# ai2cm/pace

Hardware: AMD Instinct MI355X
Metric: cell-updates/s per acoustic substep (d_sw+riem3), C192x79L; % HBM roofline (higher is better)
Workload: dtype f64; 1 GPU; C192x79L one tile per GPU, d_sw + riem_solver3 acoustic substep, fp64; cells_per_tile=2912256, tiles=1, parallelism=tile-per-gpu x1, halo_exchange=none, launch=eager, streams=one stream

## Files before the change

pace_amd/csrc/k_fxadv.hip:

```cpp
#include "common.h"
#include "kernels.h"

typedef SplitBox FxBox;

__device__ __forceinline__ double contra(double v1, double v2, double cosa, double rsin2) {
  return (v1 - v2 * cosa) * rsin2;
}

__device__ __forceinline__ void fx_vt_edges_point(const Geo& g, const Met& m, const real* vc, const real* ut, real* vt, int i, int j,
                                                  int k) {
  if (i > g.ni - 2 || j > g.nj - 2) return;
  const long c = IDX3(g, i, j, k);
  const long c2 = IDX2(g, i, j);
  if (j == g.js || j == g.je + 1) {
    const double v = vc[c];
    vt[c] = (v > 0.0) ? (v / m.sin_sg4[c2 - g.sj]) : (v / m.sin_sg2[c2]);
    return;
  }
  const bool strip = (i == g.is - 1 || i == g.is || i == g.ie || i == g.ie + 1);
  if (strip && j >= g.js + 2 && j <= g.je - 1) {
    const double ub = 0.25 * (ut[c - g.sj] + ut[c + 1 - g.sj] + ut[c] + ut[c + 1]);
    vt[c] = contra(vc[c], ub, m.cosa_v[c2], 1.0);
  }
}

__device__ __forceinline__ void fx_ut_edges_corners_point(const Geo& g, const Met& m, const real* uc, const real* vc, real* ut,
                                                          const real* vt, int i, int j, int k) {
  if (i < 1 || j < 1 || i > g.ni - 2 || j > g.nj - 2) return;
  const long c = IDX3(g, i, j, k);
  const long c2 = IDX2(g, i, j);
  const int sj = g.sj;
  const bool rows = (j == g.js - 1 || j == g.js || j == g.je || j == g.je + 1);
  if (rows && i >= g.is + 2 && i <= g.ie - 1) {
    const double vb = 0.25 * (vt[c - 1] + vt[c] + vt[c - 1 + sj] + vt[c + sj]);
    ut[c] = contra(uc[c], vb, m.cosa_u[c2], 1.0);
    return;
  }
  if (rows && (i == g.is + 1 || i == g.ie)) {
    const double cu = m.cosa_u[c2];
    double damp, val;
    if (i == g.is + 1 && (j == g.js - 1 || j == g.je)) {
      const double cv = m.cosa_v[c2 - 1];
      damp = 1.0 / (1.0 - 0.0625 * cu * cv);
      val = (uc[c] - 0.25 * cu * (vt[c - 1 + sj] + vt[c + sj] + vt[c] + vc[c - 1] -
                                  0.25 * cv * (ut[c - 1] + ut[c - 1 - sj] + ut[c - sj]))) * damp;
    } else if (i == g.is + 1) {
      const double cv = m.cosa_v[c2 - 1 + sj];
      damp = 1.0 / (1.0 - 0.0625 * cu * cv);
      val = (uc[c] - 0.25 * cu * (vt[c - 1] + vt[c] + vt[c + sj] + vc[c - 1 + sj] -
                                  0.25 * cv * (ut[c - 1] + ut[c - 1 + sj] + ut[c + sj]))) * damp;
    } else if (j == g.js - 1 || j == g.je) {
      const double cv = m.cosa_v[c2];
      damp = 1.0 / (1.0 - 0.0625 * cu * cv);
      val = (uc[c] - 0.25 * cu * (vt[c + sj] + vt[c - 1 + sj] + vt[c - 1] + vc[c] -
                                  0.25 * cv * (ut[c + 1] + ut[c + 1 - sj] + ut[c - sj]))) * damp;
    } else {
      const double cv = m.cosa_v[c2 + sj];
      damp = 1.0 / (1.0 - 0.0625 * cu * cv);
      val = (uc[c] - 0.25 * cu * (vt[c] + vt[c - 1] + vt[c - 1 + sj] + vc[c + sj] -
                                  0.25 * cv * (ut[c + 1] + ut[c + 1 + sj] + ut[c + sj]))) * damp;
    }
    ut[c] = val;
    return;
  }
}

__device__ __forceinline__ void fx_vt_corners_point(const Geo& g, const Met& m, const real* uc, const real* vc, const real* ut,
                                                    real* vt, int i, int j, int k) {
  if (i < 1 || j < 1 || i > g.ni - 2 || j > g.nj - 2) return;
  const bool cols = (i == g.is - 1 || i == g.is || i == g.ie || i == g.ie + 1);
  if (!cols || !(j == g.js + 1 || j == g.je)) return;
  const long c = IDX3(g, i, j, k);
  const long c2 = IDX2(g, i, j);
  const int sj = g.sj;
  const double cv = m.cosa_v[c2];
  double damp, val;
  if (j == g.js + 1 && (i == g.is - 1 || i == g.ie)) {
    const double cu = m.cosa_u[c2 - sj];
    damp = 1.0 / (1.0 - 0.0625 * cu * cv);
    val = (vc[c] - 0.25 * cv * (ut[c + 1 - sj] + ut[c + 1] + ut[c] + uc[c - sj] -
                                0.25 * cu * (vt[c - sj] + vt[c - 1 - sj] + vt[c - 1]))) * damp;
  } else if (j == g.js + 1) {
    const double cu = m.cosa_u[c2 + 1 - sj];
    damp = 1.0 / (1.0 - 0.0625 * cu * cv);
    val = (vc[c] - 0.25 * cv * (ut[c - sj] + ut[c] + ut[c + 1] + uc[c + 1 - sj] -
                                0.25 * cu * (vt[c - sj] + vt[c + 1 - sj] + vt[c + 1]))) * damp;
  } else if (i == g.ie + 1 || i == g.is) {
    const double cu = m.cosa_u[c2 + 1];
    damp = 1.0 / (1.0 - 0.0625 * cu * cv);
    val = (vc[c] - 0.25 * cv * (ut[c] + ut[c - sj] + ut[c + 1 - sj] + uc[c + 1] -
                                0.25 * cu * (vt[c + sj] + vt[c + 1 + sj] + vt[c + 1]))) * damp;
  } else {
    const double cu = m.cosa_u[c2];
    damp = 1.0 / (1.0 - 0.0625 * cu * cv);
    val = (vc[c] - 0.25 * cv * (ut[c + 1] + ut[c + 1 - sj] + ut[c - sj] + uc[c] -
                                0.25 * cu * (vt[c + sj] + vt[c - 1 + sj] + vt[c - 1]))) * damp;
  }
  vt[c] = val;
}

struct FxStrips {
  Regions b, c, d;
};
__device__ __forceinline__ bool strip_point(const Regions& R, int p, int& i, int& j) {
  for (int q = 0; q < R.n; ++q) {
    const int w = R.ie[q] - R.ib[q] + 1, h = R.je[q] - R.jb[q] + 1;
    if (p < w * h) {
      j = R.jb[q] + p / w;
      i = R.ib[q] + p % w;
      return true;
    }
    p -= w * h;
  }
  return false;
}
__device__ __forceinline__ int strip_count(const Regions& R) {
  int n = 0;
  for (int q = 0; q < R.n; ++q) n += (R.ie[q] - R.ib[q] + 1) * (R.je[q] - R.jb[q] + 1);
  return n;
}
struct FxFramePointA {
  long c;
  bool xedge, umain, vmain;
  double u0, u_s, u1_s, u1, v0, v_1, v_1s, vs, s3, s1, cu, ru, cv, rv;
  __device__ __forceinline__ void load(const Geo& g, const Met& m, const real* __restrict__ uc, const real* __restrict__ vc, bool on, int i,
                                       int j, int k) {
    const long c2 = IDX2(g, i, j);
    c = IDX3(g, i, j, k);
    const int sj = g.sj;
    xedge = on && (i == g.is || i == g.ie + 1);
    umain = on && !xedge && i >= g.is - 1 && i <= g.ie + 2 && !(j == g.js - 1 || j == g.js || j == g.je || j == g.je + 1);
    vmain = on && j >= g.js - 1 && j <= g.je + 2;
    u0 = u_s = u1_s = u1 = v0 = v_1 = v_1s = vs = s3 = s1 = cu = ru = cv = rv = 0.0;
    if (xedge || umain || vmain) u0 = uc[c];
    if (umain || vmain) v0 = vc[c];
    if (xedge) s3 = m.sin_sg3[c2 - 1], s1 = m.sin_sg1[c2];
    if (umain) v_1 = vc[c - 1], v_1s = vc[c - 1 + sj], vs = vc[c + sj], cu = m.cosa_u[c2], ru = m.rsin_u[c2];
    if (vmain) u_s = uc[c - sj], u1_s = uc[c + 1 - sj], u1 = uc[c + 1], cv = m.cosa_v[c2], rv = m.rsin_v[c2];
  }
  __device__ __forceinline__ void finish(real* ut, real* vt) const {
    if (xedge) {
      ut[c] = (u0 > 0.0) ? (u0 / s3) : (u0 / s1);
    } else if (umain) {
      const double vb = 0.25 * (v_1 + v0 + v_1s + vs);
      ut[c] = contra(u0, vb, cu, ru);
    }
    if (vmain) {
      const double ub = 0.25 * (u_s + u1_s + u0 + u1);
      vt[c] = contra(v0, ub, cv, rv);
    }
  }
};
struct FxFramePointF {
  long c;
  bool do_x, do_y;
  double u, v, rdxa_m, rdxa_0, dy, sg3_m, sg1_0, rdya_m, rdya_0, dx, sg4_m, sg2_0, cxa, cya;
  __device__ __forceinline__ void load(const Geo& g, const Met& m, const real* ut, const real* vt, const real* cx_acc, const real* cy_acc,
                                       bool on, int i, int j, int k) {
    const long c2 = IDX2(g, i, j);
    c = c2 + (long)k * g.sk;
    const int sj = g.sj;
    do_x = on && i >= g.is && i <= g.ie + 1, do_y = on && j >= g.js && j <= g.je + 1;
    u = v = rdxa_m = rdxa_0 = dy = sg3_m = sg1_0 = rdya_m = rdya_0 = dx = sg4_m = sg2_0 = cxa = cya = 0.0;
    if (do_x) {
      u = ut[c], rdxa_m = m.rdxa[c2 - 1], rdxa_0 = m.rdxa[c2], dy = m.dy[c2], sg3_m = m.sin_sg3[c2 - 1], sg1_0 = m.sin_sg1[c2];
      if (cx_acc) cxa = cx_acc[c];
    }
    if (do_y) {
      v = vt[c], rdya_m = m.rdya[c2 - sj], rdya_0 = m.rdya[c2], dx = m.dx[c2], sg4_m = m.sin_sg4[c2 - sj], sg2_0 = m.sin_sg2[c2];
      if (cy_acc) cya = cy_acc[c];
    }
  }
  __device__ __forceinline__ void finish(double dt, real* crx, real* cry, real* xfx, real* yfx, real* cx_acc, real* cy_acc) const {
    if (do_x) {
      double cr;
      if (u > 0.0) {
        cr = dt * u * rdxa_m;
        xfx[c] = dy * dt * u * sg3_m;
      } else {
        cr = dt * u * rdxa_0;
        xfx[c] = dy * dt * u * sg1_0;
      }
      crx[c] = cr;
      if (cx_acc) cx_acc[c] = cxa + cr;
    }
    if (do_y) {
      double cr;
      if (v > 0.0) {
        cr = dt * v * rdya_m;
        yfx[c] = dx * dt * v * sg4_m;
      } else {
        cr = dt * v * rdya_0;
        yfx[c] = dx * dt * v * sg2_0;
      }
      cry[c] = cr;
      if (cy_acc) cy_acc[c] = cya + cr;
    }
  }
};
#ifndef FX_NB
#define FX_NB 1
#endif

#ifndef FX_NT
#define FX_NT 1024
#endif
#ifndef FX_MIN_WGS
#define FX_MIN_WGS (512 * 1024 / FX_NT)
#endif
#ifndef FX_ATTR
#define FX_ATTR
#endif
template <int FXC>
__global__ void __launch_bounds__(FX_NT) FX_ATTR k_fxadv_fused(Geo g, Met m, const real* __restrict__ uc, const real* __restrict__ vc, real* ut, real* vt,
                                                      real* __restrict__ crx, real* __restrict__ cry, real* __restrict__ xfx,
                                                      real* __restrict__ yfx, double dt, real* __restrict__ cx_acc,
                                                      real* __restrict__ cy_acc, FxBox box, int contra_out, Regions A, FxStrips S,
                                                      int nframe, int nbx, FxWindHalo wh) {
  const int tid = (int)threadIdx.x;
  int b = (int)blockIdx.x;
  if (b < nframe) {
    const int k = b;
    int i, j;
    const int na = strip_count(A);
    if (wh.u_out != nullptr)
      for (int p = tid, n = wind_halo_points(g); p < n; p += FX_NT) wind_halo_copy_point(g, p, k, wh.u, wh.v, wh.u_out, wh.v_out);
    for (int p0 = tid; p0 < na; p0 += FX_NT * FX_NB) {
      FxFramePointA P[FX_NB];
#pragma unroll
      for (int q = 0; q < FX_NB; ++q) {
        int pi = 0, pj = 0;
        const bool on = strip_point(A, p0 + q * FX_NT, pi, pj) && pi <= g.ni - 2 && pj <= g.nj - 2;
        P[q].load(g, m, uc, vc, on, on ? pi : 1, on ? pj : 1, k);
      }
#pragma unroll
      for (int q = 0; q < FX_NB; ++q) P[q].finish(ut, vt);
    }
    __threadfence_block();
    __syncthreads();
    for (int p = tid, n = strip_count(S.b); p < n; p += FX_NT)
      if (strip_point(S.b, p, i, j)) fx_vt_edges_point(g, m, vc, ut, vt, i, j, k);
    __threadfence_block();
    __syncthreads();
    for (int p = tid, n = strip_count(S.c); p < n; p += FX_NT)
      if (strip_point(S.c, p, i, j)) fx_ut_edges_corners_point(g, m, uc, vc, ut, vt, i, j, k);
    __threadfence_block();
    __syncthreads();
    for (int p = tid, n = strip_count(S.d); p < n; p += FX_NT)
      if (strip_point(S.d, p, i, j)) fx_vt_corners_point(g, m, uc, vc, ut, vt, i, j, k);
    __threadfence_block();
    __syncthreads();
    for (int p0 = tid; p0 < na; p0 += FX_NT * FX_NB) {
      FxFramePointF P[FX_NB];
#pragma unroll
      for (int q = 0; q < FX_NB; ++q) {
        int pi = 0, pj = 0;
        const bool on = strip_point(A, p0 + q * FX_NT, pi, pj);
        P[q].load(g, m, ut, vt, cx_acc, cy_acc, on, on ? pi : 1, on ? pj : 1, k);
      }
#pragma unroll
      for (int q = 0; q < FX_NB; ++q) P[q].finish(dt, crx, cry, xfx, yfx, cx_acc, cy_acc);
    }
    return;
  }
  b -= nframe;
#ifdef PACE_EMU
  const int chunk = b / nbx, bxp = b - chunk * nbx;
#else
  const int seg = nbx / 8;
  const int chunk = b / nbx, r = b - chunk * nbx;
  const int bxp = (r & 7) * seg + (r >> 3);
#endif
  const long p = (long)bxp * FX_NT + tid;
  const int j = (int)(p / g.sj);
  const int i = (int)(p - (long)j * g.sj);
  if (i < box.i0 || i > box.i1 || j < box.j0 || j > box.j1) return;
  const int k0 = chunk * FXC;
  const long c2 = IDX2(g, i, j);
  const int sj = g.sj;
  const double rdxa_m = m.rdxa[c2 - 1], rdxa_0 = m.rdxa[c2], dy = m.dy[c2], sg3_m = m.sin_sg3[c2 - 1], sg1_0 = m.sin_sg1[c2];
  const double rdya_m = m.rdya[c2 - sj], rdya_0 = m.rdya[c2], dx = m.dx[c2], sg4_m = m.sin_sg4[c2 - sj], sg2_0 = m.sin_sg2[c2];
  const double cosa_u = m.cosa_u[c2], rsin_u = m.rsin_u[c2], cosa_v = m.cosa_v[c2], rsin_v = m.rsin_v[c2];
#pragma unroll
  for (int t = 0; t < FXC; ++t) {
    const int k = k0 + t;
    if (k >= g.nk) break;
    const long c = c2 + (long)k * g.sk;
    const double uc0 = uc[c], vc0 = vc[c];
    const double vb = 0.25 * (vc[c - 1] + vc0 + vc[c - 1 + sj] + vc[c + sj]);
    const double ub = 0.25 * (uc[c - sj] + uc[c + 1 - sj] + uc0 + uc[c + 1]);
    const double u = contra(uc0, vb, cosa_u, rsin_u);
    const double v = contra(vc0, ub, cosa_v, rsin_v);
    if (contra_out) ut[c] = u, vt[c] = v;
    double cr;
    if (u > 0.0) {
      cr = dt * u * rdxa_m;
      xfx[c] = dy * dt * u * sg3_m;
    } else {
      cr = dt * u * rdxa_0;
      xfx[c] = dy * dt * u * sg1_0;
    }
    crx[c] = cr;
    if (cx_acc) cx_acc[c] = cx_acc[c] + cr;
    if (v > 0.0) {
      cr = dt * v * rdya_m;
      yfx[c] = dx * dt * v * sg4_m;
    } else {
      cr = dt * v * rdya_0;
      yfx[c] = dx * dt * v * sg2_0;
    }
    cry[c] = cr;
    if (cy_acc) cy_acc[c] = cy_acc[c] + cr;
  }
}

static void fxadv_frame_regions(const Geo& g, bool has_box, Regions& A, FxStrips& S) {
  if (has_box) {
    add_region(A, 0, g.ni - 2, 0, g.js + 1);
    add_region(A, 0, g.ni - 2, g.je - 1, g.nj - 2);
    add_region(A, 0, g.is + 1, g.js + 2, g.je - 2);
    add_region(A, g.ie - 1, g.ni - 2, g.js + 2, g.je - 2);
  } else {
    add_region(A, 0, g.ni - 2, 0, g.nj - 2);
  }
  add_region(S.b, 0, g.ni - 2, g.js, g.js);
  add_region(S.b, 0, g.ni - 2, g.je + 1, g.je + 1);
  add_region(S.b, g.is - 1, g.is, g.js + 2, g.je - 1);
  add_region(S.b, g.ie, g.ie + 1, g.js + 2, g.je - 1);
  add_region(S.c, g.is + 1, g.ie, g.js - 1, g.js);
  add_region(S.c, g.is + 1, g.ie, g.je, g.je + 1);
  add_region(S.d, g.is - 1, g.ie + 1, g.js + 1, g.js + 1);
  add_region(S.d, g.is - 1, g.ie + 1, g.je, g.je);
}

int launch_fxadv(const Geo& g, const Met& m, const real* uc, const real* vc, real* crx, real* cry,
                 real* xfx, real* yfx, real* ut, real* vt, double dt, real* cx_acc, real* cy_acc,
                 hipStream_t st, int part, int contra_out, FxWindHalo* wind_halo) {
  FxBox box{g.is + 2, g.ie - 2, g.js + 2, g.je - 2, part};
  const bool has_box = box.i1 >= box.i0 && box.j1 >= box.j0;
  if (!has_box) box.i1 = box.i0 - 1, box.j1 = box.j0 - 1;
  if (part == 1 && !has_box) return PACE_OK;
  Regions A{};
  FxStrips S{};
  if (part != 1) fxadv_frame_regions(g, has_box, A, S);
  const int nframe = (part != 1) ? g.nk : 0;
  unsigned nbx = (unsigned)(((long)g.sj * g.nj + FX_NT - 1) / FX_NT);
#ifndef PACE_EMU
  nbx = (nbx + 7) / 8 * 8;
#endif
  const bool interior = has_box && part != 2;
  int ch = 8;
  while (ch > 1 && nbx * (unsigned)((g.nk + ch - 1) / ch) < (unsigned)FX_MIN_WGS) ch >>= 1;
  const unsigned nint = interior ? nbx * (unsigned)((g.nk + ch - 1) / ch) : 0u;
  if (nframe + nint == 0) return PACE_OK;
  FxWindHalo wcopy{nullptr, nullptr, nullptr, nullptr, false};
  if (wind_halo != nullptr && nframe > 0) wcopy = *wind_halo, wind_halo->done = true;
#define FX_GO(CH)                                                                                                                            \
  hipLaunchKernelGGL(k_fxadv_fused<CH>, dim3((unsigned)nframe + nint), dim3(FX_NT), 0, st, g, m, uc, vc, ut, vt, crx, cry, xfx, yfx, dt, cx_acc, \
                     cy_acc, box, contra_out, A, S, nframe, (int)nbx, wcopy)
  if (ch == 8) FX_GO(8);
  else if (ch == 4) FX_GO(4);
  else if (ch == 2) FX_GO(2);
  else FX_GO(1);
#undef FX_GO
  PACE_CHECK_LAUNCH();
  return PACE_OK;
}
```

pace_amd/csrc/kernels.h:

```cpp
#pragma once
#include "common.h"

struct FxWindHalo {
  const real *u, *v;
  real *u_out, *v_out;
  bool done;
};
int launch_fxadv(const Geo& g, const Met& m, const real* uc, const real* vc, real* crx, real* cry,
                 real* xfx, real* yfx, real* ut, real* vt, double dt, real* cx_acc, real* cy_acc,
                 hipStream_t st, int part = 0, int contra_out = 0, FxWindHalo* wind_halo = nullptr);
__device__ __forceinline__ void wind_halo_copy_point(const Geo& g, int p, int k, const real* __restrict__ u, const real* __restrict__ v,
                                                     real* __restrict__ u_out, real* __restrict__ v_out) {
  const int nsouth = g.js, nnorth = g.nj - 1 - g.je, nmid = g.je - g.js + 1, nwest = g.is, neast = g.ni - 1 - g.ie;
  const int rows = (nsouth + nnorth) * g.ni;
  int i, j;
  if (p < rows) {
    const int r = p / g.ni;
    i = p - r * g.ni, j = r < nsouth ? r : g.je + 1 + (r - nsouth);
  } else {
    p -= rows;
    const int w = nwest + neast, r = p / w, c = p - r * w;
    if (r >= nmid) return;
    j = g.js + r, i = c < nwest ? c : g.ie + 1 + (c - nwest);
  }
  const long ch = IDX3(g, i, j, k);
  const bool in_i = i >= g.is && i <= g.ie, in_j = j >= g.js && j <= g.je;
  if (!(in_i && (in_j || j == g.je + 1))) u_out[ch] = u[ch];
  if (!((in_i || i == g.ie + 1) && in_j)) v_out[ch] = v[ch];
}
__host__ __device__ __forceinline__ int wind_halo_points(const Geo& g) {
  return (g.js + g.nj - 1 - g.je) * g.ni + (g.je - g.js + 1) * (g.is + g.ni - 1 - g.ie);
}
int launch_fvtp2d(const Geo& g, const Met& m, const real* q, const real* crx, const real* cry,
                  const real* xfx, const real* yfx, real* fx, real* fy, const real* xmf,
                  const real* ymf, int hord, int nlev, hipStream_t st);
struct FvDamp {
  const real* damp_k;
  const real* nord_k;
  const real* mass;
  real* fx2o;
  real* fy2o;
  int nmax, mass_given;
  real* qout;
  const real* amass;
  real* dw;
  real* heat_s;
  real* diss_est;
  const real* damp_w_k;
  const real* ke_bg_k;
  double dt;
  real* accx;
  real* accy;
  const real* add2d;
  real* u_upd;
  real* v_upd;
  const real* ke;
  real* u_out;
  real* v_out;
};

int launch_transport(const Geo& g, const Met& m, const real* q, const real* crx, const real* cry, const real* xfx,
                     const real* yfx, real* fx, real* fy, const real* xmf, const real* ymf, int hord, int nlev,
                     int dmode, int epi, const FvDamp& dp, hipStream_t st);
int launch_transport_scalars3(const Geo& g, const Met& m, const real* w, const real* q_con, const real* pt, const real* crx,
                              const real* cry, const real* xfx, const real* yfx, const real* xmf, const real* ymf, int nlev,
                              const FvDamp& dpw, const FvDamp& dpq, const FvDamp& dpt, hipStream_t st);
int launch_transport_lean(const Geo& g, const Met& m, const real* q, const real* crx, const real* cry, const real* xfx,
                          const real* yfx, real* fx, real* fy, const real* xu, const real* yu, int hord, int nlev, int dmode,
                          int epi, const FvDamp& dp, hipStream_t st);

struct DswWinds {
  const real *rel_vort, *u, *v, *ke, *vort_b;
  real *u_out, *v_out, *heat_source;
  int do_skeb, copy_halo;
  int ke_plus_vort;
  double d_con;
};
bool dsw_scalars_take_winds();
int launch_dsw_scalars_lean(const Geo& g, const Met& m, const real* delp, const real* pt, const real* w, const real* q_con,
                            real* const* outs, const real* crx, const real* cry, const real* xfx, const real* yfx, real* mfx,
                            real* mfy, real* dw, real* heat_s, real* diss_est, const real* kc, int hord, int nmax_v, int nmax_w,
                            int nmax_t, double dt, hipStream_t st, const DswWinds* winds = nullptr);
bool transport_lean_covers(const Geo& g, int hord);

struct FvMet {
  const real *area, *rarea, *dxa, *dya, *dx, *dy, *del6_u, *del6_v;
};
static inline FvMet fv_met(const Met& m) { return FvMet{m.area, m.rarea, m.dxa, m.dya, m.dx, m.dy, m.del6_u, m.del6_v}; }

struct FvTile {
  int bx, by, bz;
};
__device__ __forceinline__ FvTile fv_tile_of_workgroup() {
#ifdef PACE_EMU
  return FvTile{(int)blockIdx.x, (int)blockIdx.y, (int)blockIdx.z};
#else
  const int gx = gridDim.x, gy = gridDim.y, nlev = gridDim.z;
  const int tpl = gx * gy;
  const int b = blockIdx.x + gx * (blockIdx.y + gy * blockIdx.z);
  const int full = (nlev / 8) * 8;
  int lev, t;
  if (b < full * tpl) {
    const int xcd = b & 7, slot = b >> 3;
    lev = (slot / tpl) * 8 + xcd;
    t = slot - (slot / tpl) * tpl;
  } else {
    lev = b / tpl;
    t = b - lev * tpl;
  }
  if (gx >= 3 && gy >= 3) {
    if (t < 4) return FvTile{(t & 1) ? gx - 1 : 0, (t & 2) ? gy - 1 : 0, lev};
    t -= 4;
    const int nsn = 2 * (gx - 2), nwe = 2 * (gy - 2);
    if (t < nsn) return FvTile{1 + (t >> 1), (t & 1) ? gy - 1 : 0, lev};
    t -= nsn;
    if (t < nwe) return FvTile{(t & 1) ? gx - 1 : 0, 1 + (t >> 1), lev};
    t -= nwe;
    return FvTile{1 + t % (gx - 2), 1 + t / (gx - 2), lev};
  }
  return FvTile{t % gx, t / gx, lev};
#endif
}
int launch_delnflux(const Geo& g, const Met& m, int mode, const real* q, real* fx, real* fy,
                    const real* mass, const real* damp_k, const real* nord_k, int nmax, int mass_given,
                    int nlev, hipStream_t st);
int launch_a2b_ord4(const Geo& g, const Met& m, real* qin, real* qout, int k0, int k1, int replace, hipStream_t st);
int launch_a2b_ord4_tiled(const Geo& g, const Met& m, const real* qin, real* qout, int k0, int k1, hipStream_t st);
int launch_a2b_ord4_batch(const Geo& g, const Met& m, const real* const* qin, real* const* qout, const int* k0, const int* k1,
                          int nfields, hipStream_t st);
int64_t dsw_workspace_bytes(const Geo& g);
bool dsw_pingpong_supported(const Geo& g, const pace_dsw_config_t* cfg);
bool dsw_winds_in_scalars(const Geo& g, const pace_dsw_config_t* cfg);
int dsw_prepare(const Geo& g, const pace_column_t* col, void* ws, hipStream_t st);
int launch_d_sw(const Geo& g, const Met& m, const pace_column_t* col, const pace_dsw_config_t* cfg, void* ws,
                real* delpc, real* delp, real* pt, real* u, real* v, real* w, real* uc, real* vc,
                const real* ua, const real* va, real* divgd, real* mfx, real* mfy, real* cx, real* cy,
                real* crx, real* cry, real* xfx, real* yfx, real* q_con, const real* zh,
                real* heat_source, real* diss_est, double dt, int phases, hipStream_t st);
int64_t riem3_workspace_bytes(const Geo& g);
int launch_riem_solver3(const Geo& g, void* ws, int last_call, double dt, const real* cappa, double ptop,
                        const real* zs, const real* wsd, real* delz, const real* q_con, const real* delp,
                        const real* pt, real* zh, real* pe, real* ppe, real* pk3, real* pk, real* peln,
                        real* w, double p_fac, hipStream_t st);
int launch_ppm1d(const Geo& g, const Met& m, int axis, int iord, const real* q, const real* c, real* out, int i0, int j0,
                 int k0, int ni, int nj, int nk, hipStream_t st);
int launch_divergence_damping(const Geo& g, const Met& m, const real* u, const real* v, const real* va, real* vort_b,
                              const real* ua, real* divg_d, real* vc, real* uc, real* delpc, real* ke,
                              const real* rel_vort_agrid, double dt, const real* d2_bg_dev, int kstart, int nonzero_nord,
                              double dddmp, double d4_bg, real* da, real* db, hipStream_t st, bool skip_dead = false,
                              bool ke_by_consumer = false, const int* ddh_tab = nullptr);
bool riem_column_supported(const Geo& g);
int launch_riem_solver3_column(const Geo& g, int last_call, double dt, const real* cappa, double ptop, const real* zs,
                               const real* wsd, real* delz, const real* q_con, const real* delp, const real* pt,
                               real* zh, real* pe, real* ppe, real* pk3, real* pk, real* peln, real* w,
                               double p_fac, hipStream_t st);
int launch_riem_solver_c_column(const Geo& g, double dt2, const real* cappa, double ptop, const real* hs, const real* ws3,
                                const real* ptc, const real* q_con, const real* delpc, real* gz, real* pef,
                                const real* w3, double p_fac, hipStream_t st);
int64_t sim1_workspace_bytes(const Geo& g);
int launch_sim1_solver(const Geo& g, void* ws, int n_halo, double dt, double p_fac, const real* gamma, const real* cp3,
                       real* pe, const real* delta_mass, const real* pm, const real* pem, real* w, real* dz,
                       const real* pt, const real* ws2d, hipStream_t st);
int64_t csw_workspace_bytes(const Geo& g);
int launch_d2a2c_vect(const Geo& g, const Met& m, void* ws, real* uc, real* vc, const real* u, const real* v,
                      real* ua, real* va, real* utc, real* vtc, hipStream_t st);
int launch_c_sw(const Geo& g, const Met& m, void* ws, real* delpc, real* ptc, real* delp, real* pt,
                const real* u, const real* v, real* w, real* uc, real* vc, real* ua, real* va,
                real* ut, real* vt, real* divgd, real* omga, double dt2, int nord, hipStream_t st, int part = 0);
int64_t riemc_workspace_bytes(const Geo& g);
int launch_riem_solver_c(const Geo& g, void* ws, double dt2, const real* cappa, double ptop, const real* hs,
                         const real* ws3, const real* ptc, const real* q_con, const real* delpc, real* gz,
                         real* pef, const real* w3, double p_fac, hipStream_t st);
int64_t updatedzc_workspace_bytes(const Geo& g);
int launch_updatedzc(const Geo& g, const Met& m, void* ws_, const real* dp_ref, const real* zs, const real* ut,
                     const real* vt, real* gz, real* ws, double dt, hipStream_t st);
int64_t updatedzd_workspace_bytes(const Geo& g);
int launch_updatedzd(const Geo& g, const Met& m, void* ws_, const pace_updatedzd_k_t* kc, const real* zs, real* zh,
                     const real* crx, const real* cry, const real* xfx, const real* yfx, real* wsd, double dt,
                     int hord_tm, hipStream_t st);
int launch_gz_from_surface(const Geo& g, const real* zs, const real* delz, real* gz, hipStream_t st);
int launch_scale_copy(const Geo& g, const real* src, real* dst, double factor, int scale, int halo, int nlev,
                      hipStream_t st);
int launch_p_grad_c(const Geo& g, const Met& m, real* uc, real* vc, const real* delpc, const real* pkc,
                    const real* gz, double dt2, hipStream_t st);
int64_t nh_p_grad_workspace_bytes(const Geo& g);
int launch_nh_p_grad(const Geo& g, const Met& m, void* ws_, real* u, real* v, real* pp, real* gz, real* pk3,
                     real* delp, double dt, double ptop, double akap, hipStream_t st);
int launch_edge_pe(const Geo& g, real* pe, const real* delp, double ptop, hipStream_t st);
int launch_pk3_halo(const Geo& g, real* pk3, const real* delp, double ptop, double akap, hipStream_t st);
int launch_ray_fast(const Geo& g, real* u, real* v, real* w, const double* dp, const double* pfull, double dt,
                    double ptop, double rf_cutoff, double tau, int hydrostatic, hipStream_t st);
int64_t del2cubed_workspace_bytes(const Geo& g);
int launch_del2cubed(const Geo& g, const Met& m, void* ws_, real* qdel, double cd, int nmax, hipStream_t st);
int launch_diffusive_heating(const Geo& g, const real* delp, const real* delz, const real* cappa,
                             const real* heat_source, real* pt, double delt_time_factor, int nlev, hipStream_t st);
int launch_halo_copy(const Geo& g, const pace_halo_desc_t* descs, int ndesc, int unpack, hipStream_t st);
int launch_tracer_flux_compute(const Geo& g, const Met& m, const real* cx, const real* cy, real* xfx, real* yfx,
                               hipStream_t st);
int launch_tracer_divide(const Geo& g, real* cxd, real* xfx, real* mfxd, real* cyd, real* yfx, real* mfyd,
                         int n_split, hipStream_t st);
int launch_apply_mass_flux(const Geo& g, const Met& m, const real* dp1, const real* mfx, const real* mfy, real* dp2,
                           hipStream_t st);
int launch_apply_tracer_flux(const Geo& g, const Met& m, real* q, const real* dp1, const real* fx, const real* fy,
                             const real* dp2, hipStream_t st);
int64_t map_single_workspace_bytes(const Geo& g, int nq);
int launch_map_fields(const Geo& g, void* ws, real* const* q, int nq, const real* pe1, const real* pe2, const real* qs,
                      double qmin, int kord, int iv, int xstag, int ystag, hipStream_t st);
int launch_fillz(const Geo& g, real* const* q, int nq, const real* dp, hipStream_t st);
int launch_l2e_prepare(const Geo& g, const real* const* water, real* q_con, real* pt, real* cappa, real* delp,
                       real* delz, const real* pe, real* pe1, real* pe2, const real* ak, const real* bk, real* dp2,
                       real* ps, real* pn2, const real* peln, real* pk, double ptop, double akap, double r_vir,
                       hipStream_t st);
int launch_l2e_post(const Geo& g, const real* const* water, real* q_con, real* pkz, const real* pt, real* cappa,
                    const real* delp, real* delz, real* peln, real* pe0, const real* pn2, double r_vir, hipStream_t st);
int launch_l2e_pressures(const Geo& g, int dir, const real* pe, const real* pe1, const real* ak, const real* bk,
                         real* pe0, real* pe3, hipStream_t st);
int launch_l2e_finish(const Geo& g, const real* const* water, real* pe, const real* pe2, real* pt, const real* pkz,
                      double r_vir, int last_step, hipStream_t st);
int launch_sat_adjust_tables(double* tables, hipStream_t st);
int launch_sat_adjust(const Geo& g, real* const* water, real* qcld, real* te, real* pt, real* q_con, real* pkz, real* cappa,
                      const real* delp, const real* delz, const real* area, const real* hs, const double* tables,
                      const pace_sat_adjust_params_t& p, int kmp, int last_step, int consv_te, hipStream_t st);

int launch_dry_convective_adjust(const Geo& g, real* const* tracers, real* pt, real* ua, real* va, real* w, real* u_dt,
                                 real* v_dt, const real* delp, const real* delz, const real* pkz, const real* peln,
                                 const real* pe, int k_sponge, double xvir, double t_max, double fv_sg_adj, double timestep,
                                 hipStream_t st);
int launch_fill_gfs_delp(const Geo& g, const real* delp, real* q, double q_min, hipStream_t st);
int launch_phys_thermo_pressure(const Geo& g, const real* const* water, real* pt, real* t_dt, real* pe, const real* delp,
                                real* peln, real* pk, const real* ua, const real* va, real* ps, real* u_srf, real* v_srf,
                                double dt, hipStream_t st);
int launch_update_dwinds_phys(const Geo& g, real* u, real* v, real* u_dt, real* v_dt, const real* const* vlon,
                              const real* const* vlat, const real* const* es1, const real* const* ew2, const real* edge_vect_w,
                              const real* edge_vect_e, const real* edge_vect_s, const real* edge_vect_n, double dt5,
                              hipStream_t st);
long microphysics_workspace_bytes(const Geo& g);
int launch_microphysics(const Geo& g, void* workspace, const real* const* in, real* wmp, real* const* tend, real* const* precip,
                        const pace_microphysics_config_t& cfg, hipStream_t st);
int launch_copy_dycore_to_physics(const Geo& g, const real* const* in, real* const* out, hipStream_t st);
int launch_physics_prepare(const Geo& g, real* const* tracers, const real* pt, const real* delz, real* delp, const real* omga,
                           real* prsi, real* phii, real* phil, real* delprsi, real* dz, real* wmp, real* const* tendencies,
                           double ptop, int do_microphysics, hipStream_t st);
int launch_physics_update_state(const Geo& g, const real* const* x, const real* const* x_dt, real* const* out, double dt,
                                hipStream_t st);
int launch_physics_tendencies_to_dycore(const Geo& g, real* const* tendencies, const real* const* updated,
                                        const real* const* before, real* const* tracers, const real* prsi, real* delp,
                                        double rdt, hipStream_t st);
int launch_fv_setup_pt(const Geo& g, real* const* water, real* q_con, real* pkz, real* pt, real* cappa,
                       const real* delp, const real* delz, real* dp1, hipStream_t st);
int launch_omega_from_w(const Geo& g, const real* delp, const real* delz, const real* w, real* omga, hipStream_t st);
int launch_neg_adj3(const Geo& g, real* const* water, real* qcld, real* pt, const real* delp, hipStream_t st);
int launch_c2l(const Geo& g, const Met& m, int order, const real* u, const real* v, const real* a11, const real* a12,
               const real* a21, const real* a22, real* ua, real* va, hipStream_t st);
int launch_stencil(const Geo& g, const Met& m, int id, void* const* fields, int nfields, const double* scalars, int nscalars,
                   const int* origin, const int* domain, hipStream_t st);
int launch_swap_dp(const Geo& g, real* dp1, real* dp2, hipStream_t st);
int launch_zero_data(const Geo& g, real* mfxd, real* mfyd, real* cxd, real* cyd, real* heat_source, real* diss_estd,
                     int first_timestep, hipStream_t st);
int launch_interface_pressure(const Geo& g, const real* delp, real* pem, double ptop, hipStream_t st);
```

Measured before the change: 4.061 billion cell-updates/s.

## Tile fxadv frame into shared-memory segments per level instead of one workgroup per level

```diff
diff --git a/pace_amd/csrc/k_fxadv.hip b/pace_amd/csrc/k_fxadv.hip
--- a/pace_amd/csrc/k_fxadv.hip
+++ b/pace_amd/csrc/k_fxadv.hip
@@ -7,171 +7,191 @@
   return (v1 - v2 * cosa) * rsin2;
 }
 
-__device__ __forceinline__ void fx_vt_edges_point(const Geo& g, const Met& m, const real* vc, const real* ut, real* vt, int i, int j,
-                                                  int k) {
-  if (i > g.ni - 2 || j > g.nj - 2) return;
-  const long c = IDX3(g, i, j, k);
+#ifndef FX_NT
+#define FX_NT 1024
+#endif
+#ifndef FX_SEG
+#define FX_SEG 104
+#endif
+#define FX_THICK 5
+#define FX_TILE ((FX_THICK + 4) * (FX_SEG + 4))
+#define FX_WIND ((FX_THICK + 2) * (FX_SEG + 2))
+static_assert(FX_TILE <= FX_NT, "a frame workgroup loads one point of uc / vc per thread");
+struct FxFrame {
+  int n;
+  int i0[4], i1[4], j0[4], j1[4];
+  int alongx[4];
+  int first[5];
+};
+
+__device__ __forceinline__ void fx_frame_segment(const Geo& g, const Met& m, const real* __restrict__ uc, const real* __restrict__ vc,
+                                                 real* __restrict__ ut, real* __restrict__ vt, real* __restrict__ crx,
+                                                 real* __restrict__ cry, real* __restrict__ xfx, real* __restrict__ yfx, double dt,
+                                                 real* __restrict__ cx_acc, real* __restrict__ cy_acc, const FxFrame& F, int k, int w,
+                                                 const FxWindHalo& wh) {
+  __shared__ double s_uc[FX_TILE], s_vc[FX_TILE], s_ut[FX_WIND], s_vt[FX_WIND];
+  const int tid = (int)threadIdx.x;
+  const int sj = g.sj;
+  int q = 0;
+  while (q + 1 < F.n && w >= F.first[q + 1]) ++q;
+  int oi0 = F.i0[q], oi1 = F.i1[q], oj0 = F.j0[q], oj1 = F.j1[q];
+  {
+    const int s = w - F.first[q], nseg = F.first[q + 1] - F.first[q];
+    if (F.alongx[q]) {
+      const int len = (oi1 - oi0 + nseg) / nseg;
+      oi0 += s * len;
+      oi1 = oi1 < oi0 + len - 1 ? oi1 : oi0 + len - 1;
+    } else {
+      const int len = (oj1 - oj0 + nseg) / nseg;
+      oj0 += s * len;
+      oj1 = oj1 < oj0 + len - 1 ? oj1 : oj0 + len - 1;
+    }
+  }
+  const int ai0 = oi0 > 0 ? oi0 - 1 : 0, ai1 = oi1 + 1 < g.ni - 2 ? oi1 + 1 : g.ni - 2;
+  const int aj0 = oj0 > 0 ? oj0 - 1 : 0, aj1 = oj1 + 1 < g.nj - 2 ? oj1 + 1 : g.nj - 2;
+  const int ti0 = oi0 > 1 ? oi0 - 2 : 0, ti1 = oi1 + 2 < g.ni - 1 ? oi1 + 2 : g.ni - 1;
+  const int tj0 = oj0 > 1 ? oj0 - 2 : 0, tj1 = oj1 + 2 < g.nj - 1 ? oj1 + 2 : g.nj - 1;
+  const int ow = oi1 - oi0 + 1, oh = oj1 - oj0 + 1, aw = ai1 - ai0 + 1, ah = aj1 - aj0 + 1, tw = ti1 - ti0 + 1, th = tj1 - tj0 + 1;
+
+  double uc_t = 0.0, vc_t = 0.0;
+  if (tid < tw * th) {
+    const int tj = tid / tw, ti = tid - tj * tw;
+    const long c = IDX3(g, ti0 + ti, tj0 + tj, k);
+    uc_t = uc[c], vc_t = vc[c];
+  }
+  const bool a_on = tid < aw * ah;
+  const int a_j = aj0 + (a_on ? tid / aw : 0), a_i = ai0 + (a_on ? tid % aw : 0);
+  const bool a_rows = (a_j == g.js - 1 || a_j == g.js || a_j == g.je || a_j == g.je + 1);
+  const bool a_xedge = a_on && (a_i == g.is || a_i == g.ie + 1);
+  const bool a_umain = a_on && !a_xedge && a_i >= g.is - 1 && a_i <= g.ie + 2 && !a_rows;
+  const bool a_yedge = a_on && (a_j == g.js || a_j == g.je + 1);
+  const bool a_vmain = a_on && !a_yedge && a_j >= g.js - 1 && a_j <= g.je + 2;
+  double a_u0 = 0.0, a_u1 = 0.0, a_v0 = 0.0, a_v1 = 0.0;
+  {
+    const long c2 = IDX2(g, a_i, a_j);
+    if (a_xedge) a_u0 = m.sin_sg3[c2 - 1], a_u1 = m.sin_sg1[c2];
+    if (a_umain) a_u0 = m.cosa_u[c2], a_u1 = m.rsin_u[c2];
+    if (a_yedge) a_v0 = m.sin_sg4[c2 - sj], a_v1 = m.sin_sg2[c2];
+    if (a_vmain) a_v0 = m.cosa_v[c2], a_v1 = m.rsin_v[c2];
+  }
+  const bool o_on = tid < ow * oh;
+  const int j = oj0 + (o_on ? tid / ow : 0), i = oi0 + (o_on ? tid % ow : 0);
   const long c2 = IDX2(g, i, j);
-  if (j == g.js || j == g.je + 1) {
-    const double v = vc[c];
-    vt[c] = (v > 0.0) ? (v / m.sin_sg4[c2 - g.sj]) : (v / m.sin_sg2[c2]);
-    return;
-  }
-  const bool strip = (i == g.is - 1 || i == g.is || i == g.ie || i == g.ie + 1);
-  if (strip && j >= g.js + 2 && j <= g.je - 1) {
-    const double ub = 0.25 * (ut[c - g.sj] + ut[c + 1 - g.sj] + ut[c] + ut[c + 1]);
-    vt[c] = contra(vc[c], ub, m.cosa_v[c2], 1.0);
-  }
-}
-
-__device__ __forceinline__ void fx_ut_edges_corners_point(const Geo& g, const Met& m, const real* uc, const real* vc, real* ut,
-                                                          const real* vt, int i, int j, int k) {
-  if (i < 1 || j < 1 || i > g.ni - 2 || j > g.nj - 2) return;
-  const long c = IDX3(g, i, j, k);
-  const long c2 = IDX2(g, i, j);
-  const int sj = g.sj;
+  const long c = c2 + (long)k * g.sk;
   const bool rows = (j == g.js - 1 || j == g.js || j == g.je || j == g.je + 1);
-  if (rows && i >= g.is + 2 && i <= g.ie - 1) {
-    const double vb = 0.25 * (vt[c - 1] + vt[c] + vt[c - 1 + sj] + vt[c + sj]);
-    ut[c] = contra(uc[c], vb, m.cosa_u[c2], 1.0);
-    return;
-  }
-  if (rows && (i == g.is + 1 || i == g.ie)) {
-    const double cu = m.cosa_u[c2];
-    double damp, val;
-    if (i == g.is + 1 && (j == g.js - 1 || j == g.je)) {
-      const double cv = m.cosa_v[c2 - 1];
-      damp = 1.0 / (1.0 - 0.0625 * cu * cv);
-      val = (uc[c] - 0.25 * cu * (vt[c - 1 + sj] + vt[c + sj] + vt[c] + vc[c - 1] -
-                                  0.25 * cv * (ut[c - 1] + ut[c - 1 - sj] + ut[c - sj]))) * damp;
-    } else if (i == g.is + 1) {
-      const double cv = m.cosa_v[c2 - 1 + sj];
-      damp = 1.0 / (1.0 - 0.0625 * cu * cv);
-      val = (uc[c] - 0.25 * cu * (vt[c - 1] + vt[c] + vt[c + sj] + vc[c - 1 + sj] -
-                                  0.25 * cv * (ut[c - 1] + ut[c - 1 + sj] + ut[c + sj]))) * damp;
-    } else if (j == g.js - 1 || j == g.je) {
-      const double cv = m.cosa_v[c2];
-      damp = 1.0 / (1.0 - 0.0625 * cu * cv);
-      val = (uc[c] - 0.25 * cu * (vt[c + sj] + vt[c - 1 + sj] + vt[c - 1] + vc[c] -
-                                  0.25 * cv * (ut[c + 1] + ut[c + 1 - sj] + ut[c - sj]))) * damp;
+  const bool cols = (i == g.is - 1 || i == g.is || i == g.ie || i == g.ie + 1);
+  const bool xedge = (i == g.is || i == g.ie + 1);
+  const bool umain = !xedge && i >= g.is - 1 && i <= g.ie + 2 && !rows;
+  const bool c_main = o_on && rows && i >= g.is + 2 && i <= g.ie - 1;
+  const bool c_corner = o_on && !c_main && rows && (i == g.is + 1 || i == g.ie);
+  const bool b_col = o_on && !(j == g.js || j == g.je + 1) && cols && j >= g.js + 2 && j <= g.je - 1;
+  const bool d_pt = o_on && cols && (j == g.js + 1 || j == g.je);
+  const bool put_u = o_on && (xedge || umain || c_main || c_corner);
+  const bool put_v = o_on && j >= g.js - 1 && j <= g.je + 2;
+  const bool lo_row = (j == g.js - 1 || j == g.je);
+  double o_cu = 0.0, o_cv = 0.0;
+  if (c_main) o_cu = m.cosa_u[c2];
+  if (c_corner) {
+    o_cu = m.cosa_u[c2];
+    o_cv = m.cosa_v[c2 + (i == g.is + 1 ? -1 : 0) + (lo_row ? 0 : sj)];
+  }
+  if (b_col) o_cv = m.cosa_v[c2];
+  if (d_pt) {
+    o_cv = m.cosa_v[c2];
+    if (j == g.js + 1) o_cu = m.cosa_u[c2 - sj + ((i == g.is - 1 || i == g.ie) ? 0 : 1)];
+    else o_cu = m.cosa_u[c2 + ((i == g.ie + 1 || i == g.is) ? 1 : 0)];
+  }
+  const bool do_x = o_on && i >= g.is && i <= g.ie + 1, do_y = o_on && j >= g.js && j <= g.je + 1;
+  double rdxa_m = 0.0, rdxa_0 = 0.0, dy = 0.0, sg3_m = 0.0, sg1_0 = 0.0, rdya_m = 0.0, rdya_0 = 0.0, dx = 0.0, sg4_m = 0.0, sg2_0 = 0.0,
+         cxa = 0.0, cya = 0.0;
+  if (do_x) {
+    rdxa_m = m.rdxa[c2 - 1], rdxa_0 = m.rdxa[c2], dy = m.dy[c2], sg3_m = m.sin_sg3[c2 - 1], sg1_0 = m.sin_sg1[c2];
+    if (cx_acc) cxa = cx_acc[c];
+  }
+  if (do_y) {
+    rdya_m = m.rdya[c2 - sj], rdya_0 = m.rdya[c2], dx = m.dx[c2], sg4_m = m.sin_sg4[c2 - sj], sg2_0 = m.sin_sg2[c2];
+    if (cy_acc) cya = cy_acc[c];
+  }
+  const int nwl = F.first[F.n];
+  long wc = 0;
+  bool w_u = false, w_v = false;
+  real w_uv = 0, w_vv = 0;
+  if (wh.u_out != nullptr) {
+    const int p = w * FX_NT + tid;
+    if (p < wind_halo_points(g) && wind_halo_index(g, p, k, wc, w_u, w_v)) {
+      if (w_u) w_uv = wh.u[wc];
+      if (w_v) w_vv = wh.v[wc];
     } else {
-      const double cv = m.cosa_v[c2 + sj];
-      damp = 1.0 / (1.0 - 0.0625 * cu * cv);
-      val = (uc[c] - 0.25 * cu * (vt[c] + vt[c - 1] + vt[c - 1 + sj] + vc[c + sj] -
-                                  0.25 * cv * (ut[c + 1] + ut[c + 1 + sj] + ut[c + sj]))) * damp;
-    }
-    ut[c] = val;
-    return;
-  }
-}
-
-__device__ __forceinline__ void fx_vt_corners_point(const Geo& g, const Met& m, const real* uc, const real* vc, const real* ut,
-                                                    real* vt, int i, int j, int k) {
-  if (i < 1 || j < 1 || i > g.ni - 2 || j > g.nj - 2) return;
-  const bool cols = (i == g.is - 1 || i == g.is || i == g.ie || i == g.ie + 1);
-  if (!cols || !(j == g.js + 1 || j == g.je)) return;
-  const long c = IDX3(g, i, j, k);
-  const long c2 = IDX2(g, i, j);
-  const int sj = g.sj;
-  const double cv = m.cosa_v[c2];
-  double damp, val;
-  if (j == g.js + 1 && (i == g.is - 1 || i == g.ie)) {
-    const double cu = m.cosa_u[c2 - sj];
-    damp = 1.0 / (1.0 - 0.0625 * cu * cv);
-    val = (vc[c] - 0.25 * cv * (ut[c + 1 - sj] + ut[c + 1] + ut[c] + uc[c - sj] -
-                                0.25 * cu * (vt[c - sj] + vt[c - 1 - sj] + vt[c - 1]))) * damp;
-  } else if (j == g.js + 1) {
-    const double cu = m.cosa_u[c2 + 1 - sj];
-    damp = 1.0 / (1.0 - 0.0625 * cu * cv);
-    val = (vc[c] - 0.25 * cv * (ut[c - sj] + ut[c] + ut[c + 1] + uc[c + 1 - sj] -
-                                0.25 * cu * (vt[c - sj] + vt[c + 1 - sj] + vt[c + 1]))) * damp;
-  } else if (i == g.ie + 1 || i == g.is) {
-    const double cu = m.cosa_u[c2 + 1];
-    damp = 1.0 / (1.0 - 0.0625 * cu * cv);
-    val = (vc[c] - 0.25 * cv * (ut[c] + ut[c - sj] + ut[c + 1 - sj] + uc[c + 1] -
-                                0.25 * cu * (vt[c + sj] + vt[c + 1 + sj] + vt[c + 1]))) * damp;
-  } else {
-    const double cu = m.cosa_u[c2];
-    damp = 1.0 / (1.0 - 0.0625 * cu * cv);
-    val = (vc[c] - 0.25 * cv * (ut[c + 1] + ut[c + 1 - sj] + ut[c - sj] + uc[c] -
-                                0.25 * cu * (vt[c + sj] + vt[c - 1 + sj] + vt[c - 1]))) * damp;
-  }
-  vt[c] = val;
-}
-
-struct FxStrips {
-  Regions b, c, d;
-};
-__device__ __forceinline__ bool strip_point(const Regions& R, int p, int& i, int& j) {
-  for (int q = 0; q < R.n; ++q) {
-    const int w = R.ie[q] - R.ib[q] + 1, h = R.je[q] - R.jb[q] + 1;
-    if (p < w * h) {
-      j = R.jb[q] + p / w;
-      i = R.ib[q] + p % w;
-      return true;
-    }
-    p -= w * h;
-  }
-  return false;
-}
-__device__ __forceinline__ int strip_count(const Regions& R) {
-  int n = 0;
-  for (int q = 0; q < R.n; ++q) n += (R.ie[q] - R.ib[q] + 1) * (R.je[q] - R.jb[q] + 1);
-  return n;
-}
-struct FxFramePointA {
-  long c;
-  bool xedge, umain, vmain;
-  double u0, u_s, u1_s, u1, v0, v_1, v_1s, vs, s3, s1, cu, ru, cv, rv;
-  __device__ __forceinline__ void load(const Geo& g, const Met& m, const real* __restrict__ uc, const real* __restrict__ vc, bool on, int i,
-                                       int j, int k) {
-    const long c2 = IDX2(g, i, j);
-    c = IDX3(g, i, j, k);
-    const int sj = g.sj;
-    xedge = on && (i == g.is || i == g.ie + 1);
-    umain = on && !xedge && i >= g.is - 1 && i <= g.ie + 2 && !(j == g.js - 1 || j == g.js || j == g.je || j == g.je + 1);
-    vmain = on && j >= g.js - 1 && j <= g.je + 2;
-    u0 = u_s = u1_s = u1 = v0 = v_1 = v_1s = vs = s3 = s1 = cu = ru = cv = rv = 0.0;
-    if (xedge || umain || vmain) u0 = uc[c];
-    if (umain || vmain) v0 = vc[c];
-    if (xedge) s3 = m.sin_sg3[c2 - 1], s1 = m.sin_sg1[c2];
-    if (umain) v_1 = vc[c - 1], v_1s = vc[c - 1 + sj], vs = vc[c + sj], cu = m.cosa_u[c2], ru = m.rsin_u[c2];
-    if (vmain) u_s = uc[c - sj], u1_s = uc[c + 1 - sj], u1 = uc[c + 1], cv = m.cosa_v[c2], rv = m.rsin_v[c2];
-  }
-  __device__ __forceinline__ void finish(real* ut, real* vt) const {
-    if (xedge) {
-      ut[c] = (u0 > 0.0) ? (u0 / s3) : (u0 / s1);
-    } else if (umain) {
-      const double vb = 0.25 * (v_1 + v0 + v_1s + vs);
-      ut[c] = contra(u0, vb, cu, ru);
-    }
-    if (vmain) {
-      const double ub = 0.25 * (u_s + u1_s + u0 + u1);
-      vt[c] = contra(v0, ub, cv, rv);
-    }
-  }
-};
-struct FxFramePointF {
-  long c;
-  bool do_x, do_y;
-  double u, v, rdxa_m, rdxa_0, dy, sg3_m, sg1_0, rdya_m, rdya_0, dx, sg4_m, sg2_0, cxa, cya;
-  __device__ __forceinline__ void load(const Geo& g, const Met& m, const real* ut, const real* vt, const real* cx_acc, const real* cy_acc,
-                                       bool on, int i, int j, int k) {
-    const long c2 = IDX2(g, i, j);
-    c = c2 + (long)k * g.sk;
-    const int sj = g.sj;
-    do_x = on && i >= g.is && i <= g.ie + 1, do_y = on && j >= g.js && j <= g.je + 1;
-    u = v = rdxa_m = rdxa_0 = dy = sg3_m = sg1_0 = rdya_m = rdya_0 = dx = sg4_m = sg2_0 = cxa = cya = 0.0;
-    if (do_x) {
-      u = ut[c], rdxa_m = m.rdxa[c2 - 1], rdxa_0 = m.rdxa[c2], dy = m.dy[c2], sg3_m = m.sin_sg3[c2 - 1], sg1_0 = m.sin_sg1[c2];
-      if (cx_acc) cxa = cx_acc[c];
-    }
-    if (do_y) {
-      v = vt[c], rdya_m = m.rdya[c2 - sj], rdya_0 = m.rdya[c2], dx = m.dx[c2], sg4_m = m.sin_sg4[c2 - sj], sg2_0 = m.sin_sg2[c2];
-      if (cy_acc) cya = cy_acc[c];
-    }
-  }
-  __device__ __forceinline__ void finish(double dt, real* crx, real* cry, real* xfx, real* yfx, real* cx_acc, real* cy_acc) const {
+      w_u = w_v = false;
+    }
+  }
+
+  if (tid < tw * th) s_uc[tid] = uc_t, s_vc[tid] = vc_t;
+  __syncthreads();
+  if (a_on) {
+    const int t = (a_i - ti0) + (a_j - tj0) * tw;
+    const double u0 = s_uc[t], v0 = s_vc[t];
+    if (a_xedge) {
+      s_ut[tid] = (u0 > 0.0) ? (u0 / a_u0) : (u0 / a_u1);
+    } else if (a_umain) {
+      const double vb = 0.25 * (s_vc[t - 1] + v0 + s_vc[t - 1 + tw] + s_vc[t + tw]);
+      s_ut[tid] = contra(u0, vb, a_u0, a_u1);
+    }
+    if (a_yedge) {
+      s_vt[tid] = (v0 > 0.0) ? (v0 / a_v0) : (v0 / a_v1);
+    } else if (a_vmain) {
+      const double ub = 0.25 * (s_uc[t - tw] + s_uc[t + 1 - tw] + u0 + s_uc[t + 1]);
+      s_vt[tid] = contra(v0, ub, a_v0, a_v1);
+    }
+  }
+  __syncthreads();
+
+  if (o_on) {
+    const int a = (i - ai0) + (j - aj0) * aw;
+    const int t = (i - ti0) + (j - tj0) * tw;
+    const double* const UT = s_ut + a;
+    const double* const VT = s_vt + a;
+    const double* const UC = s_uc + t;
+    const double* const VC = s_vc + t;
+    double u = 0.0, v = 0.0;
+    if (c_main) {
+      const double vb = 0.25 * (VT[-1] + VT[0] + VT[-1 + aw] + VT[aw]);
+      u = contra(UC[0], vb, o_cu, 1.0);
+    } else if (c_corner) {
+      const double cu = o_cu, cv = o_cv;
+      const double damp = 1.0 / (1.0 - 0.0625 * cu * cv);
+      if (i == g.is + 1 && lo_row) {
+        u = (UC[0] - 0.25 * cu * (VT[-1 + aw] + VT[aw] + VT[0] + VC[-1] - 0.25 * cv * (UT[-1] + UT[-1 - aw] + UT[-aw]))) * damp;
+      } else if (i == g.is + 1) {
+        u = (UC[0] - 0.25 * cu * (VT[-1] + VT[0] + VT[aw] + VC[-1 + tw] - 0.25 * cv * (UT[-1] + UT[-1 + aw] + UT[aw]))) * damp;
+      } else if (lo_row) {
+        u = (UC[0] - 0.25 * cu * (VT[aw] + VT[-1 + aw] + VT[-1] + VC[0] - 0.25 * cv * (UT[1] + UT[1 - aw] + UT[-aw]))) * damp;
+      } else {
+        u = (UC[0] - 0.25 * cu * (VT[0] + VT[-1] + VT[-1 + aw] + VC[tw] - 0.25 * cv * (UT[1] + UT[1 + aw] + UT[aw]))) * damp;
+      }
+    } else if (put_u) {
+      u = UT[0];
+    }
+    if (b_col) {
+      const double ub = 0.25 * (UT[-aw] + UT[1 - aw] + UT[0] + UT[1]);
+      v = contra(VC[0], ub, o_cv, 1.0);
+    } else if (d_pt) {
+      const double cu = o_cu, cv = o_cv;
+      const double damp = 1.0 / (1.0 - 0.0625 * cu * cv);
+      if (j == g.js + 1 && (i == g.is - 1 || i == g.ie)) {
+        v = (VC[0] - 0.25 * cv * (UT[1 - aw] + UT[1] + UT[0] + UC[-tw] - 0.25 * cu * (VT[-aw] + VT[-1 - aw] + VT[-1]))) * damp;
+      } else if (j == g.js + 1) {
+        v = (VC[0] - 0.25 * cv * (UT[-aw] + UT[0] + UT[1] + UC[1 - tw] - 0.25 * cu * (VT[-aw] + VT[1 - aw] + VT[1]))) * damp;
+      } else if (i == g.ie + 1 || i == g.is) {
+        v = (VC[0] - 0.25 * cv * (UT[0] + UT[-aw] + UT[1 - aw] + UC[1] - 0.25 * cu * (VT[aw] + VT[1 + aw] + VT[1]))) * damp;
+      } else {
+        v = (VC[0] - 0.25 * cv * (UT[1] + UT[1 - aw] + UT[-aw] + UC[0] - 0.25 * cu * (VT[aw] + VT[-1 + aw] + VT[-1]))) * damp;
+      }
+    } else if (put_v) {
+      v = VT[0];
+    }
+    if (put_u) ut[c] = u;
+    if (put_v) vt[c] = v;
     if (do_x) {
       double cr;
       if (u > 0.0) {
@@ -197,14 +217,13 @@
       if (cy_acc) cy_acc[c] = cya + cr;
     }
   }
-};
-#ifndef FX_NB
-#define FX_NB 1
-#endif
-
-#ifndef FX_NT
-#define FX_NT 1024
-#endif
+  if (w_u) wh.u_out[wc] = w_uv;
+  if (w_v) wh.v_out[wc] = w_vv;
+  if (wh.u_out != nullptr)
+    for (int p = (nwl + w) * FX_NT + tid, n = wind_halo_points(g); p < n; p += nwl * FX_NT)
+      wind_halo_copy_point(g, p, k, wh.u, wh.v, wh.u_out, wh.v_out);
+}
+
 #ifndef FX_MIN_WGS
 #define FX_MIN_WGS (512 * 1024 / FX_NT)
 #endif
@@ -215,52 +234,13 @@
 __global__ void __launch_bounds__(FX_NT) FX_ATTR k_fxadv_fused(Geo g, Met m, const real* __restrict__ uc, const real* __restrict__ vc, real* ut, real* vt,
                                                       real* __restrict__ crx, real* __restrict__ cry, real* __restrict__ xfx,
                                                       real* __restrict__ yfx, double dt, real* __restrict__ cx_acc,
-                                                      real* __restrict__ cy_acc, FxBox box, int contra_out, Regions A, FxStrips S,
+                                                      real* __restrict__ cy_acc, FxBox box, int contra_out, FxFrame F,
                                                       int nframe, int nbx, FxWindHalo wh) {
   const int tid = (int)threadIdx.x;
   int b = (int)blockIdx.x;
   if (b < nframe) {
-    const int k = b;
-    int i, j;
-    const int na = strip_count(A);
-    if (wh.u_out != nullptr)
-      for (int p = tid, n = wind_halo_points(g); p < n; p += FX_NT) wind_halo_copy_point(g, p, k, wh.u, wh.v, wh.u_out, wh.v_out);
-    for (int p0 = tid; p0 < na; p0 += FX_NT * FX_NB) {
-      FxFramePointA P[FX_NB];
-#pragma unroll
-      for (int q = 0; q < FX_NB; ++q) {
-        int pi = 0, pj = 0;
-        const bool on = strip_point(A, p0 + q * FX_NT, pi, pj) && pi <= g.ni - 2 && pj <= g.nj - 2;
-        P[q].load(g, m, uc, vc, on, on ? pi : 1, on ? pj : 1, k);
-      }
-#pragma unroll
-      for (int q = 0; q < FX_NB; ++q) P[q].finish(ut, vt);
-    }
-    __threadfence_block();
-    __syncthreads();
-    for (int p = tid, n = strip_count(S.b); p < n; p += FX_NT)
-      if (strip_point(S.b, p, i, j)) fx_vt_edges_point(g, m, vc, ut, vt, i, j, k);
-    __threadfence_block();
-    __syncthreads();
-    for (int p = tid, n = strip_count(S.c); p < n; p += FX_NT)
-      if (strip_point(S.c, p, i, j)) fx_ut_edges_corners_point(g, m, uc, vc, ut, vt, i, j, k);
-    __threadfence_block();
-    __syncthreads();
-    for (int p = tid, n = strip_count(S.d); p < n; p += FX_NT)
-      if (strip_point(S.d, p, i, j)) fx_vt_corners_point(g, m, uc, vc, ut, vt, i, j, k);
-    __threadfence_block();
-    __syncthreads();
-    for (int p0 = tid; p0 < na; p0 += FX_NT * FX_NB) {
-      FxFramePointF P[FX_NB];
-#pragma unroll
-      for (int q = 0; q < FX_NB; ++q) {
-        int pi = 0, pj = 0;
-        const bool on = strip_point(A, p0 + q * FX_NT, pi, pj);
-        P[q].load(g, m, ut, vt, cx_acc, cy_acc, on, on ? pi : 1, on ? pj : 1, k);
-      }
-#pragma unroll
-      for (int q = 0; q < FX_NB; ++q) P[q].finish(dt, crx, cry, xfx, yfx, cx_acc, cy_acc);
-    }
+    const int nwl = F.first[F.n], k = b / nwl;
+    fx_frame_segment(g, m, uc, vc, ut, vt, crx, cry, xfx, yfx, dt, cx_acc, cy_acc, F, k, b - k * nwl, wh);
     return;
   }
   b -= nframe;
@@ -314,36 +294,33 @@
   }
 }
 
-static void fxadv_frame_regions(const Geo& g, bool has_box, Regions& A, FxStrips& S) {
-  if (has_box) {
-    add_region(A, 0, g.ni - 2, 0, g.js + 1);
-    add_region(A, 0, g.ni - 2, g.je - 1, g.nj - 2);
-    add_region(A, 0, g.is + 1, g.js + 2, g.je - 2);
-    add_region(A, g.ie - 1, g.ni - 2, g.js + 2, g.je - 2);
-  } else {
-    add_region(A, 0, g.ni - 2, 0, g.nj - 2);
-  }
-  add_region(S.b, 0, g.ni - 2, g.js, g.js);
-  add_region(S.b, 0, g.ni - 2, g.je + 1, g.je + 1);
-  add_region(S.b, g.is - 1, g.is, g.js + 2, g.je - 1);
-  add_region(S.b, g.ie, g.ie + 1, g.js + 2, g.je - 1);
-  add_region(S.c, g.is + 1, g.ie, g.js - 1, g.js);
-  add_region(S.c, g.is + 1, g.ie, g.je, g.je + 1);
-  add_region(S.d, g.is - 1, g.ie + 1, g.js + 1, g.js + 1);
-  add_region(S.d, g.is - 1, g.ie + 1, g.je, g.je);
+static void fx_add_strip(FxFrame& F, int i0, int i1, int j0, int j1, bool alongx) {
+  if (i1 < i0 || j1 < j0) return;
+  const int q = F.n++;
+  F.i0[q] = i0, F.i1[q] = i1, F.j0[q] = j0, F.j1[q] = j1, F.alongx[q] = alongx;
+  const int len = alongx ? i1 - i0 + 1 : j1 - j0 + 1;
+  F.first[q + 1] = F.first[q] + (len + FX_SEG - 1) / FX_SEG;
+}
+static FxFrame fxadv_frame_regions(const Geo& g) {
+  FxFrame F{};
+  const int n0 = g.je - 1 > g.js + 2 ? g.je - 1 : g.js + 2;
+  fx_add_strip(F, 0, g.ni - 2, 0, g.js + 1, true);
+  fx_add_strip(F, 0, g.ni - 2, n0, g.nj - 2, true);
+  fx_add_strip(F, 0, g.is + 1, g.js + 2, g.je - 2, false);
+  fx_add_strip(F, g.ie - 1, g.ni - 2, g.js + 2, g.je - 2, false);
+  return F;
 }
 
 int launch_fxadv(const Geo& g, const Met& m, const real* uc, const real* vc, real* crx, real* cry,
                  real* xfx, real* yfx, real* ut, real* vt, double dt, real* cx_acc, real* cy_acc,
                  hipStream_t st, int part, int contra_out, FxWindHalo* wind_halo) {
+  if (g.n < 3) return PACE_ERR_UNSUPPORTED;
   FxBox box{g.is + 2, g.ie - 2, g.js + 2, g.je - 2, part};
   const bool has_box = box.i1 >= box.i0 && box.j1 >= box.j0;
   if (!has_box) box.i1 = box.i0 - 1, box.j1 = box.j0 - 1;
   if (part == 1 && !has_box) return PACE_OK;
-  Regions A{};
-  FxStrips S{};
-  if (part != 1) fxadv_frame_regions(g, has_box, A, S);
-  const int nframe = (part != 1) ? g.nk : 0;
+  const FxFrame F = (part != 1) ? fxadv_frame_regions(g) : FxFrame{};
+  const int nframe = g.nk * F.first[F.n];
   unsigned nbx = (unsigned)(((long)g.sj * g.nj + FX_NT - 1) / FX_NT);
 #ifndef PACE_EMU
   nbx = (nbx + 7) / 8 * 8;
@@ -357,7 +334,7 @@
   if (wind_halo != nullptr && nframe > 0) wcopy = *wind_halo, wind_halo->done = true;
 #define FX_GO(CH)                                                                                                                            \
   hipLaunchKernelGGL(k_fxadv_fused<CH>, dim3((unsigned)nframe + nint), dim3(FX_NT), 0, st, g, m, uc, vc, ut, vt, crx, cry, xfx, yfx, dt, cx_acc, \
-                     cy_acc, box, contra_out, A, S, nframe, (int)nbx, wcopy)
+                     cy_acc, box, contra_out, F, nframe, (int)nbx, wcopy)
   if (ch == 8) FX_GO(8);
   else if (ch == 4) FX_GO(4);
   else if (ch == 2) FX_GO(2);
diff --git a/pace_amd/csrc/kernels.h b/pace_amd/csrc/kernels.h
--- a/pace_amd/csrc/kernels.h
+++ b/pace_amd/csrc/kernels.h
@@ -9,8 +9,7 @@
 int launch_fxadv(const Geo& g, const Met& m, const real* uc, const real* vc, real* crx, real* cry,
                  real* xfx, real* yfx, real* ut, real* vt, double dt, real* cx_acc, real* cy_acc,
                  hipStream_t st, int part = 0, int contra_out = 0, FxWindHalo* wind_halo = nullptr);
-__device__ __forceinline__ void wind_halo_copy_point(const Geo& g, int p, int k, const real* __restrict__ u, const real* __restrict__ v,
-                                                     real* __restrict__ u_out, real* __restrict__ v_out) {
+__device__ __forceinline__ bool wind_halo_index(const Geo& g, int p, int k, long& ch, bool& copy_u, bool& copy_v) {
   const int nsouth = g.js, nnorth = g.nj - 1 - g.je, nmid = g.je - g.js + 1, nwest = g.is, neast = g.ni - 1 - g.ie;
   const int rows = (nsouth + nnorth) * g.ni;
   int i, j;
@@ -20,13 +19,22 @@
   } else {
     p -= rows;
     const int w = nwest + neast, r = p / w, c = p - r * w;
-    if (r >= nmid) return;
+    if (r >= nmid) return false;
     j = g.js + r, i = c < nwest ? c : g.ie + 1 + (c - nwest);
   }
-  const long ch = IDX3(g, i, j, k);
+  ch = IDX3(g, i, j, k);
   const bool in_i = i >= g.is && i <= g.ie, in_j = j >= g.js && j <= g.je;
-  if (!(in_i && (in_j || j == g.je + 1))) u_out[ch] = u[ch];
-  if (!((in_i || i == g.ie + 1) && in_j)) v_out[ch] = v[ch];
+  copy_u = !(in_i && (in_j || j == g.je + 1));
+  copy_v = !((in_i || i == g.ie + 1) && in_j);
+  return true;
+}
+__device__ __forceinline__ void wind_halo_copy_point(const Geo& g, int p, int k, const real* __restrict__ u, const real* __restrict__ v,
+                                                     real* __restrict__ u_out, real* __restrict__ v_out) {
+  long ch;
+  bool copy_u, copy_v;
+  if (!wind_halo_index(g, p, k, ch, copy_u, copy_v)) return;
+  if (copy_u) u_out[ch] = u[ch];
+  if (copy_v) v_out[ch] = v[ch];
 }
 __host__ __device__ __forceinline__ int wind_halo_points(const Geo& g) {
   return (g.js + g.nj - 1 - g.je) * g.ni + (g.je - g.js + 1) * (g.is + g.ni - 1 - g.ie);
```

Measured after the change: 4.055 billion cell-updates/s, median of 2. About the same (-0.1%).
